# dsforza96/yocto-hair

Measured on AMD Instinct MI355X. Metric: Msamples/sec (whole node), 720x720x1536spp sphere-hairblock; per-pixel L2 vs CPU ref, higher is better.
Workload: dtype f32

## Files before the change

### yocto-hair_amd/csrc/dev_hair.h

```cpp
#ifndef YH_DEV_HAIR_H_
#define YH_DEV_HAIR_H_
#include "dev_math.h"

namespace yhd {

constexpr int p_max = 3;

struct hair_hit {
  float h, gamma_o;
  frame w2b;
};

#ifndef YH_HAIR_FAST
#define YH_HAIR_FAST 1
#endif
#define YH_FAST_DIV YH_HAIR_FAST
#define YH_FAST_EXP 0
#define YH_FAST_LOG YH_HAIR_FAST
#define YH_FAST_TRIG YH_HAIR_FAST
#define YH_FAST_ASIN YH_HAIR_FAST
YH_DEV float h_rcp(float x) { return YH_FAST_DIV ? __builtin_amdgcn_rcpf(x) : 1 / x; }
YH_DEV float h_div(float a, float b) { return YH_FAST_DIV ? a * __builtin_amdgcn_rcpf(b) : a / b; }
YH_DEV float h_div_n(float a, float b) {
  if (!YH_FAST_DIV) return a / b;
// ... 236 lines not shown
  o.pdf0 = ap_pdf[0], o.pdf1 = ap_pdf[1], o.pdf2 = ap_pdf[2], o.pdf3 = ap_pdf[3];
  return o;
}

YH_DEV void hair_eval_pdf_quad(const yhd_material& m, const hair_hit& hh, const hair_out& ho, f3 incoming_,
    f3& f, float& pdf) {
  const int p       = (int)(__lane_id() & 3u);
  f3    incoming    = quad_normalize(transform_vector(hh.w2b, incoming_));
  float sin_theta_o = ho.sin_theta_o, cos_theta_o = ho.cos_theta_o;
  float sin_theta_i = incoming.x;
  float cos_theta_i = exact_safe_sqrt(1 - sqr(sin_theta_i));
  float phi_i       = atan2f(incoming.z, incoming.y);
  float phi         = phi_i - ho.phi_o;
  float sin_theta_op, cos_theta_op;
  tilt(m, p, sin_theta_o, cos_theta_o, sin_theta_op, cos_theta_op);
  if (p < p_max) cos_theta_op = fabs_(cos_theta_op);
  float mpv  = mp(m, p, cos_theta_i, cos_theta_op, sin_theta_i, sin_theta_op);
  float npv  = p < p_max ? np(m, phi, p, hh.gamma_o, ho.gamma_t) : 0.0f;
  const f3    a0 = ho.ap0, a1 = ho.ap1, a2 = ho.ap2, a3 = ho.ap3;
  const float q0 = ho.pdf0, q1 = ho.pdf1, q2 = ho.pdf2, q3 = ho.pdf3;
  const bool  is0 = p == 0, is1 = p == 1, is2 = p == 2;
  f3    apq  = f3{is0 ? a0.x : is1 ? a1.x : is2 ? a2.x : a3.x, is0 ? a0.y : is1 ? a1.y : is2 ? a2.y : a3.y,
      is0 ? a0.z : is1 ? a1.z : is2 ? a2.z : a3.z};
  float appq = is0 ? q0 : is1 ? q1 : is2 ? q2 : q3;
  f3    tf   = p < p_max ? mpv * apq * npv : h_div(mpv * apq, 2 * pif);
  float tp   = p < p_max ? mpv * appq * npv : mpv * appq * (1 / (2 * pif));
  f   = mk3(0.0f);
  pdf = 0.0f;
  f   = f + f3{quad_bcast_f<0>(tf.x), quad_bcast_f<0>(tf.y), quad_bcast_f<0>(tf.z)};
  pdf += quad_bcast_f<0>(tp);
  f   = f + f3{quad_bcast_f<1>(tf.x), quad_bcast_f<1>(tf.y), quad_bcast_f<1>(tf.z)};
  pdf += quad_bcast_f<1>(tp);
  f   = f + f3{quad_bcast_f<2>(tf.x), quad_bcast_f<2>(tf.y), quad_bcast_f<2>(tf.z)};
  pdf += quad_bcast_f<2>(tp);
  f   = f + f3{quad_bcast_f<3>(tf.x), quad_bcast_f<3>(tf.y), quad_bcast_f<3>(tf.z)};
  pdf += quad_bcast_f<3>(tp);
}
YH_DEV void hair_eval_pdf_lane(const yhd_material& m, const hair_hit& hh, const hair_out& ho, f3 incoming_,
    f3& f, float& pdf) {
  f3    incoming    = normalize(transform_vector(hh.w2b, incoming_));
  float sin_theta_o = ho.sin_theta_o, cos_theta_o = ho.cos_theta_o;
  float sin_theta_i = incoming.x;
  float cos_theta_i = exact_safe_sqrt(1 - sqr(sin_theta_i));
  float phi_i       = atan2f(incoming.z, incoming.y);
  float phi         = phi_i - ho.phi_o;
  f   = mk3(0.0f);
  pdf = 0.0f;
  const f3    apv[p_max]  = {ho.ap0, ho.ap1, ho.ap2};
  const float appv[p_max] = {ho.pdf0, ho.pdf1, ho.pdf2};
#pragma unroll
  for (int p = 0; p < p_max; p++) {
    float sin_theta_op, cos_theta_op;
    tilt(m, p, sin_theta_o, cos_theta_o, sin_theta_op, cos_theta_op);
    cos_theta_op = fabs_(cos_theta_op);
    float mpv    = mp(m, p, cos_theta_i, cos_theta_op, sin_theta_i, sin_theta_op);
    float npv    = np(m, phi, p, hh.gamma_o, ho.gamma_t);
    f            = f + mpv * apv[p] * npv;
    pdf += mpv * appv[p] * npv;
  }
  float mpl = mp(m, p_max, cos_theta_i, cos_theta_o, sin_theta_i, sin_theta_o);
  f         = f + h_div(mpl * ho.ap3, 2 * pif);
  pdf += mpl * ho.pdf3 * (1 / (2 * pif));
}
YH_DEV void hair_eval_pdf_quad(const yhd_material& m, const hair_hit& hh, f3 outgoing_, f3 incoming_,
    f3& f, float& pdf) {
  hair_out ho = hair_prepare<true>(m, hh, outgoing_);
  hair_eval_pdf_quad(m, hh, ho, incoming_, f, pdf);
}

YH_DEV uint32_t compact1by1(uint32_t x) {
  x &= 0x55555555;
  x = (x ^ (x >> 1)) & 0x33333333;
  x = (x ^ (x >> 2)) & 0x0f0f0f0f;
  x = (x ^ (x >> 4)) & 0x00ff00ff;
  x = (x ^ (x >> 8)) & 0x0000ffff;
  return x;
}
YH_DEV void demux_float(float f, float& a, float& b) {
  uint64_t v = (uint64_t)(f * 4294967296.0f);
  a          = (float)compact1by1((uint32_t)v) / 65536.0f;
  b          = (float)compact1by1((uint32_t)(v >> 1)) / 65536.0f;
}

YH_DEV f3 hair_sample(const yhd_material& m, const hair_hit& hh, const hair_out& ho, float rnx, float rny) {
  float sin_theta_o = ho.sin_theta_o, cos_theta_o = ho.cos_theta_o, phi_o = ho.phi_o;
  float u00, u01, u10, u11;
  demux_float(rnx, u00, u01);
  demux_float(rny, u10, u11);
  int   p  = 0;
  float u1 = u00 - ho.pdf0, u2 = u1 - ho.pdf1;
  if (!(u00 < ho.pdf0)) p = !(u1 < ho.pdf1) ? (!(u2 < ho.pdf2) ? 3 : 2) : 1;
  float sin_theta_op, cos_theta_op;
  tilt(m, p, sin_theta_o, cos_theta_o, sin_theta_op, cos_theta_op);
  u10 = fmax_(u10, 1e-5f);
  float vp = 0, em2v = 0;
  vp   = p == 0 ? m.v[0] : p == 1 ? m.v[1] : m.v[2];
  em2v = p == 0 ? m.exp_m2_inv_v[0] : p == 1 ? m.exp_m2_inv_v[1] : m.exp_m2_inv_v[2];
  float cos_theta   = 1 + vp * d_log(u10 + (1 - u10) * em2v);
  float sin_theta   = d_safe_sqrt(1 - sqr(cos_theta));
  float cos_phi     = d_cos_turns(u11);
  float sin_theta_i = -cos_theta * sin_theta_op + sin_theta * cos_phi * cos_theta_op;
  float cos_theta_i = d_safe_sqrt(1 - sqr(sin_theta_i));
  float dphi;
  if (p < p_max) {
    float x = -m.s * d_log(d_rcp(u01 * m.tl_norm + m.tl_cdf_a) - 1);
    dphi    = phi_fn(p, hh.gamma_o, ho.gamma_t) + fclamp(x, -pif, pif);
  } else {
    dphi = 2 * pif * u01;
  }
  float phi_i    = phi_o + dphi;
  f3    incoming = f3{sin_theta_i, cos_theta_i * d_cos(phi_i), cos_theta_i * d_sin(phi_i)};
  return d_transform_direction(transpose_rot(hh.w2b), incoming);
}
YH_DEV f3 hair_sample(const yhd_material& m, const hair_hit& hh, f3 outgoing_, float rnx, float rny) {
  hair_out ho = hair_prepare(m, hh, outgoing_);
  return hair_sample(m, hh, ho, rnx, rny);
}

YH_DEV void derive_material(yhd_material& m) {
#pragma unroll
  for (int p = 0; p <= p_max; p++) {
    m.inv_v[p]        = 1 / m.v[p];
    m.log_inv_2v[p]   = logf(1 / (2 * m.v[p]));
    m.exp_m2_inv_v[p] = expf(-2 / m.v[p]);
    m.mp_den[p]       = sinh((double)(1 / m.v[p])) * 2 * m.v[p];
  }
  float cb   = 1 / (1 + expf(-pif / m.s));
  float ca   = 1 / (1 + expf(-(-pif) / m.s));
  m.tl_cdf_a = ca;
  m.tl_norm  = cb - ca;
}

}
#endif
```

### yocto-hair_amd/csrc/dev_path.h

```cpp
#ifndef YH_DEV_PATH_H_
#define YH_DEV_PATH_H_
#include "dev_hair.h"
#include "dev_surface.h"
#include "dev_trace.h"
#if YH_LANE
#include "dev_lane.h"
#endif

namespace yhd {

YH_DEV ray_t sample_camera(const yhd_camera& cam, int i, int j, int w, int h, float pu, float pv,
    float lu, float lv) {
  const unsigned int ql = __lane_id() & 3u;
  float uvq = (ql == 0 ? (float)i + pu : (float)j + pv) / (ql == 0 ? (float)w : (float)h);
  float uvx = quad_bcast_f<0>(uvq), uvy = quad_bcast_f<1>(uvq);
  f3    q  = {cam.film_x * (0.5f - uvx), cam.film_y * (uvy - 0.5f), cam.lens};
  f3    dc = -quad_normalize(q);
  f3    e  = mk3(0.0f);
  if (cam.aperture != 0) {
    float r   = sqrtf(lv);
    float phi = 2 * pif * lu;
    float lx = cosf(phi) * r, ly = sinf(phi) * r;
    e = f3{lx * cam.aperture / 2, ly * cam.aperture / 2, 0};
  }
  f3    p  = quad_div(dc * cam.focus, fabs_(dc.z));
  f3    d  = quad_normalize(p - e);
  frame f  = ldframe(cam.frame);
  return mkray(transform_point(f, e), quad_normalize(transform_vector(f, d)));
}

YH_DEV ray_t sample_camera_lane(const yhd_camera& cam, int i, int j, int w, int h, float pu, float pv, float lu, float lv) {
  float uvx = ((float)i + pu) / (float)w, uvy = ((float)j + pv) / (float)h;
  f3    q   = {cam.film_x * (0.5f - uvx), cam.film_y * (uvy - 0.5f), cam.lens};
  f3    dc  = -normalize(q);
  f3    e   = mk3(0.0f);
  if (cam.aperture != 0) {
    float r   = sqrtf(lv);
    float phi = 2 * pif * lu;
    float lx = cosf(phi) * r, ly = sinf(phi) * r;
    e = f3{lx * cam.aperture / 2, ly * cam.aperture / 2, 0};
  }
  f3    p = (dc * cam.focus) / fabs_(dc.z);
  f3    d = normalize(p - e);
  frame f = ldframe(cam.frame);
  return mkray(transform_point(f, e), normalize(transform_vector(f, d)));
}

YH_DEV f3 transform_normal(const frame& a, f3 b) { return normalize(transform_vector(a, b)); }
YH_DEV f3 quad_transform_normal(const frame& a, f3 b) { return quad_normalize(transform_vector(a, b)); }

YH_DEV f3 eval_position(const yhd_scene& sc, const yhd_object& o, int element, float u, float v) {
  frame    fr = ldframe(o.frame);
  yhd_int4 e  = sc.elems[o.elem_base + element];
  if (o.kind == YH_KIND_TRIANGLES) {
    f3 p0 = xyz(sc.vpos[o.vert_base + e.x]), p1 = xyz(sc.vpos[o.vert_base + e.y]),
       p2 = xyz(sc.vpos[o.vert_base + e.z]);
    return transform_point(fr, p0 * (1 - u - v) + p1 * u + p2 * v);
  } else {
    f3 p0 = xyz(sc.vpos[o.vert_base + e.x]), p1 = xyz(sc.vpos[o.vert_base + e.y]);
    return transform_point(fr, p0 * (1 - u) + p1 * u);
  }
}

struct hit_geom {
  f3 position, normal, element_normal;
};
YH_DEV hit_geom eval_hit(const yhd_scene& sc, const yhd_object& o, int slot, float u, float v) {
  frame    fr = ldframe(o.frame);
  hit_geom g;
  if (o.kind == YH_KIND_TRIANGLES) {
    const yhd_float4* rec = sc.prims + (size_t)o.prim_base + (size_t)slot * 6;
    f3 p0 = xyz(ldg4(rec)), p1 = xyz(ldg4(rec + 1)), p2 = xyz(ldg4(rec + 2));
    g.position       = transform_point(fr, p0 * (1 - u - v) + p1 * u + p2 * v);
    g.element_normal = quad_transform_normal(fr, quad_normalize(cross(p1 - p0, p2 - p0)));
    if (o.has_normals) {
      f3 n0 = xyz(ldg4(rec + 3)), n1 = xyz(ldg4(rec + 4)), n2 = xyz(ldg4(rec + 5));
      g.normal = quad_transform_normal(fr, quad_normalize(n0 * (1 - u - v) + n1 * u + n2 * v));
    } else {
      g.normal = g.element_normal;
    }
  } else {
    const yhd_float4* rec = sc.prims + (size_t)o.prim_base + (size_t)slot * 4;
    f3 p0 = xyz(ldg4(rec)), p1 = xyz(ldg4(rec + 1));
    g.position       = transform_point(fr, p0 * (1 - u) + p1 * u);
    g.element_normal = quad_transform_normal(fr, quad_normalize(p1 - p0));
    if (o.has_normals) {
      f3 n0 = xyz(ldg4(rec + 2)), n1 = xyz(ldg4(rec + 3));
      g.normal = quad_transform_normal(fr, quad_normalize(n0 * (1 - u) + n1 * u));
    } else {
      g.normal = g.element_normal;
    }
  }
  return g;
}

YH_DEV hit_geom eval_hit_fetch_first(const yhd_scene& sc, const yhd_object& o, int slot, float u, float v) {
  const bool        tri = o.kind == YH_KIND_TRIANGLES;
  const yhd_float4* rec = sc.prims + (size_t)o.prim_base + (size_t)slot * (tri ? 6 : 4);
  const v4f r0 = ldg4(rec), r1 = ldg4(rec + 1), r2 = ldg4(rec + 2), r3 = ldg4(rec + 3);
  v4f       r4 = r3, r5 = r3;
  if (tri) r4 = ldg4(rec + 4), r5 = ldg4(rec + 5);
  frame    fr = ldframe(o.frame);
  hit_geom g;
  if (tri) {
    f3 p0 = xyz(r0), p1 = xyz(r1), p2 = xyz(r2);
    g.position       = transform_point(fr, p0 * (1 - u - v) + p1 * u + p2 * v);
    g.element_normal = quad_transform_normal(fr, quad_normalize(cross(p1 - p0, p2 - p0)));
    if (o.has_normals) {
      f3 n0 = xyz(r3), n1 = xyz(r4), n2 = xyz(r5);
      g.normal = quad_transform_normal(fr, quad_normalize(n0 * (1 - u - v) + n1 * u + n2 * v));
    } else {
      g.normal = g.element_normal;
    }
  } else {
    f3 p0 = xyz(r0), p1 = xyz(r1);
    g.position       = transform_point(fr, p0 * (1 - u) + p1 * u);
    g.element_normal = quad_transform_normal(fr, quad_normalize(p1 - p0));
    if (o.has_normals) {
      f3 n0 = xyz(r2), n1 = xyz(r3);
      g.normal = quad_transform_normal(fr, quad_normalize(n0 * (1 - u) + n1 * u));
    } else {
      g.normal = g.element_normal;
    }
  }
  return g;
}

YH_DEV f3 eval_env_texture(const yhd_scene& sc, const yhd_environment& env, float u_, float v_) {
  if (env.tex_w == 0) return mk3(1.0f);
  int   sx = env.tex_w, sy = env.tex_h;
  float s = fmodf(u_, 1.0f) * sx;
  if (s < 0) s += sx;
  float t = fmodf(v_, 1.0f) * sy;
  if (t < 0) t += sy;
  int   i = iclamp((int)s, 0, sx - 1), j = iclamp((int)t, 0, sy - 1);
  int   ii = (i + 1) % sx, jj = (j + 1) % sy;
  float u = s - i, v = t - j;
  const yhd_float4* tx = sc.env_texels + env.texel_base;
  f3 a = xyz(tx[(size_t)j * sx + i]), b = xyz(tx[(size_t)jj * sx + i]);
  f3 c = xyz(tx[(size_t)j * sx + ii]), d = xyz(tx[(size_t)jj * sx + ii]);
  return a * (1 - u) * (1 - v) + b * (1 - u) * v + c * u * (1 - v) + d * u * v;
}
template <bool COUNT, bool CENV = false>
YH_DEV f3 eval_environment(const trace_ctx& tc, f3 dir, const const_env_t* ce = nullptr) {
  const yhd_scene& sc = *tc.sc;
  f3 emission = mk3(0.0f);
  if constexpr (CENV) {
    if (COUNT)
      for (int k = 0; k < sc.num_environments; k++) count_quad<COUNT>(tc.stats->envl);
    return ld3(ce->env_sum);
  }
  for (int k = 0; k < sc.num_environments; k++) {
    const yhd_environment& env = sc.environments[k];
    if (COUNT) count_quad<COUNT>(tc.stats->envl);
    if (env.tex_w == 0) {
      emission = emission + ld3(env.emission) * mk3(1.0f);
      continue;
    }
    f3    wl = transform_direction(ldframe(env.inv_frame), dir);
    float tx = atan2f(wl.z, wl.x) / (2 * pif);
    float ty = acosf(fclamp(wl.y, -1.0f, 1.0f)) / pif;
    if (tx < 0) tx += 1;
    emission = emission + ld3(env.emission) * eval_env_texture(sc, env, tx, ty);
  }
  return emission;
}

YH_DEV void const_environments(const yhd_scene& sc, const_env_t& ce) {
  f3 emission = mk3(0.0f);
  for (int k = 0; k < sc.num_environments; k++) emission = emission + ld3(sc.environments[k].emission) * mk3(1.0f);
  float pdf = 0.0f;
  for (int k = 0; k < sc.num_lights; k++) pdf += 1 / (4 * pif);
  pdf *= (float)1 / (float)sc.num_lights;
  auto uniform = [](float v) { return __int_as_float(__builtin_amdgcn_readfirstlane(__float_as_int(v))); };
  ce.env_sum[0] = uniform(emission.x), ce.env_sum[1] = uniform(emission.y), ce.env_sum[2] = uniform(emission.z);
  ce.lights_pdf = uniform(pdf);
}

template <typename P>
YH_DEV int cdf_upper_bound(P cdf, int lo, int len, float r) {
  while (len > 0) {
    int half = len >> 1;
    if (!(r < cdf[lo + half])) {
      lo += half + 1;
      len -= half + 1;
    } else {
      len = half;
    }
  }
  return lo;
}
template <typename P>
YH_DEV int sample_discrete_cdf(P cdf, int n, float r) {
  float back = cdf[n - 1];
  r          = fclamp(r * back, 0.0f, back - 0.00001f);
  return iclamp(cdf_upper_bound(cdf, 0, n, r), 0, n - 1);
}
YH_DEV int sample_discrete_cdf_indexed(const float* cdf, int n, const YH_LDS float* tab, int K, int S, float r) {
  float back = tab[K - 1];
  r          = fclamp(r * back, 0.0f, back - 0.00001f);
  int k      = cdf_upper_bound(tab, 0, K, r);
  if (k >= K) return n - 1;
  int lo = k * S;
  return iclamp(cdf_upper_bound(cdf, lo, min(S, n - lo), r), 0, n - 1);
}

YH_DEV void object_frames(const trace_ctx& tc, int object, frame& fr, frame& inv) {
  if (tc.lds_scene) {
    const YH_LDS v4f* ob = tc.lds_scene + YH_OBJECT_F4 * object;
    v4f a = ob[0], b = ob[1], c = ob[2], d = ob[3], e = ob[4], g = ob[5];
    fr.x = {a.x, a.y, a.z}, fr.y = {a.w, b.x, b.y}, fr.z = {b.z, b.w, c.x}, fr.o = {c.y, c.z, c.w};
    inv.x = {d.x, d.y, d.z}, inv.y = {d.w, e.x, e.y}, inv.z = {e.z, e.w, g.x}, inv.o = {g.y, g.z, g.w};
  } else {
    const yhd_object& o = tc.sc->objects[object];
    fr = ldframe(o.frame), inv = ldframe(o.inv_frame);
  }
}
YH_DEV bool small_light_hit(const YH_LDS v4f* L, const frame& inv, f3 ro, f3 rd, int& slot, float& uu, float& vv) {
  f3  lo = transform_point(inv, ro), ld = transform_vector(inv, rd);
  f3  ldinv = quad_rcp(ld);
  v4f b0 = L[0], b1 = L[1];
  if (!intersect_bbox(lo, ldinv, ray_eps, flt_max, xyz(b0), xyz(b1))) return false;
  const int num  = __float_as_int(b0.w);
  float     tmax = flt_max;
  bool      hit  = false;
  for (int i = 0; i < num; i++) {
    float u = 0, v = 0, d = 0;
    if (intersect_triangle(lo, ld, ray_eps, tmax, xyz(L[2 + 3 * i]), xyz(L[3 + 3 * i]), xyz(L[4 + 3 * i]), u, v, d)) hit = true, slot = i, uu = u, vv = v, tmax = d;
  }
  return hit;
}

template <bool COUNT, bool BIG_LIGHTS, bool CENV = false>
YH_DEV f3 sample_lights(const trace_ctx& tc, f3 position, float rl, float rel, float ruvx,
    float ruvy) {
  const yhd_scene& sc = *tc.sc;
  if constexpr (CENV) {
    float z   = 2 * ruvy - 1;
    float r   = sqrtf(fclamp(1 - z * z, 0.0f, 1.0f));
    float phi = 2 * pif * ruvx;
    return f3{r * cosf(phi), r * sinf(phi), z};
  }
  int n        = sc.num_lights;
  int light_id = iclamp((int)(rl * n), 0, n - 1);
  const yhd_light& light = sc.lights[light_id];
  if (light.object >= 0 && (!BIG_LIGHTS || (light.small_base >= 0 && tc.lds_lights))) {
    const YH_LDS v4f* L = tc.lds_lights + light.small_base;
    int   element = sample_discrete_cdf((const YH_LDS float*)(L + 14), light.cdf_count, rel);
    int   rec     = 0;
    for (int i = 1; i < __float_as_int(L[0].w); i++)
      if (__float_as_int(L[2 + 3 * i].w) == element) rec = i;
    float su = sqrtf(ruvx);
    float u = 1 - su, v = ruvy * su;
    frame fr, inv;
    object_frames(tc, light.object, fr, inv);
    f3 p0 = xyz(L[2 + 3 * rec]), p1 = xyz(L[3 + 3 * rec]), p2 = xyz(L[4 + 3 * rec]);
    f3 lposition = transform_point(fr, p0 * (1 - u - v) + p1 * u + p2 * v);
    return normalize(lposition - position);
  } else if (BIG_LIGHTS && light.object >= 0) {
    int   element = sample_discrete_cdf(sc.light_cdf + light.cdf_base, light.cdf_count, rel);
    float su      = sqrtf(ruvx);
    float u = 1 - su, v = ruvy * su;
    f3 lposition = eval_position(sc, sc.objects[light.object], element, u, v);
    return normalize(lposition - position);
  } else if (light.environment >= 0) {
    const yhd_environment& env = sc.environments[light.environment];
    if (env.tex_w) {
      if (COUNT) count_quad<COUNT>(tc.stats->envs);
      int   idx = (tc.lds_envtab && light_id == sc.env_tab_light)
                      ? sample_discrete_cdf_indexed(sc.light_cdf + light.cdf_base, light.cdf_count, tc.lds_envtab, sc.env_tab_k, sc.env_tab_stride, rel)
                      : sample_discrete_cdf(sc.light_cdf + light.cdf_base, light.cdf_count, rel);
      float ux  = (idx % env.tex_w + 0.5f) / env.tex_w;
      float uy  = (idx / env.tex_w + 0.5f) / env.tex_h;
      return transform_direction(ldframe(env.frame),
          f3{cosf(ux * 2 * pif) * sinf(uy * pif), cosf(uy * pif), sinf(ux * 2 * pif) * sinf(uy * pif)});
    } else {
      float z   = 2 * ruvy - 1;
      float r   = sqrtf(fclamp(1 - z * z, 0.0f, 1.0f));
      float phi = 2 * pif * ruvx;
      return f3{r * cosf(phi), r * sinf(phi), z};
    }
  }
  return mk3(0.0f);
}

template <bool COUNT, int STRIDE, bool BIG_LIGHTS, bool CENV = false>
YH_DEV float sample_lights_pdf(const trace_ctx& tc, f3 position, f3 direction, const const_env_t* ce = nullptr) {
  const yhd_scene& sc = *tc.sc;
  float pdf = 0.0f;
  if constexpr (CENV) return ce->lights_pdf;
  for (int k = 0; k < sc.num_lights; k++) {
    const yhd_light& light = sc.lights[k];
    if (light.object >= 0 && (!BIG_LIGHTS || (light.small_base >= 0 && tc.lds_lights))) {
      const YH_LDS v4f* L = tc.lds_lights + light.small_base;
      frame fr, inv;
      object_frames(tc, light.object, fr, inv);
      const float area = L[1].w;
      float lpdf = 0.0f;
      f3    next_position = position;
      for (int bounce = 0; bounce < 100; bounce++) {
        int   slot = 0;
        float uu = 0, vv = 0;
        if (!small_light_hit(L, inv, next_position, direction, slot, uu, vv)) break;
        f3 p0 = xyz(L[2 + 3 * slot]), p1 = xyz(L[3 + 3 * slot]), p2 = xyz(L[4 + 3 * slot]);
        f3 lposition = transform_point(fr, p0 * (1 - uu - vv) + p1 * uu + p2 * vv);
        f3 lnormal   = quad_transform_normal(fr, quad_normalize(cross(p1 - p0, p2 - p0)));
        f3 dp        = lposition - position;
        lpdf += dot(dp, dp) / (fabs_(dot(lnormal, direction)) * area);
        next_position = lposition + direction * 1e-3f;
      }
      pdf += lpdf;
    } else if (BIG_LIGHTS && light.object >= 0) {
      const yhd_object& o = sc.objects[light.object];
      float lpdf = 0.0f;
      f3    next_position = position;
      for (int bounce = 0; bounce < 100; bounce++) {
        hit_t isec;
#if YH_LANE
        isec = lane_trace(tc, *tc.ls, next_position, direction, light.object);
#else
        isec = trace_ray<COUNT, STRIDE>(tc, mkray(next_position, direction), light.object);
#endif
        if (isec.object < 0) break;
        hit_geom lg        = eval_hit(sc, o, isec.slot, isec.u, isec.v);
        f3       lposition = lg.position;
        f3       lnormal   = lg.element_normal;
        float area      = sc.light_cdf[light.cdf_base + light.cdf_count - 1];
        f3    dp        = lposition - position;
        lpdf += dot(dp, dp) / (fabs_(dot(lnormal, direction)) * area);
        next_position = lposition + direction * 1e-3f;
      }
      pdf += lpdf;
    } else if (light.environment >= 0) {
      const yhd_environment& env = sc.environments[light.environment];
      if (env.tex_w) {
        f3    wl = transform_direction(ldframe(env.inv_frame), direction);
        float tx = atan2f(wl.z, wl.x) / (2 * pif);
        float ty = acosf(fclamp(wl.y, -1.0f, 1.0f)) / pif;
        if (tx < 0) tx += 1;
        int   i   = iclamp((int)(tx * env.tex_w), 0, env.tex_w - 1);
        int   j   = iclamp((int)(ty * env.tex_h), 0, env.tex_h - 1);
        int   idx = j * env.tex_w + i;
        const float* cdf = sc.light_cdf + light.cdf_base;
        float prob = (idx == 0 ? cdf[0] : cdf[idx] - cdf[idx - 1]) / cdf[light.cdf_count - 1];
        float angle = (2 * pif / env.tex_w) * (pif / env.tex_h) * sinf(pif * (j + 0.5f) / env.tex_h);
        pdf += prob / angle;
      } else {
        pdf += 1 / (4 * pif);
      }
    }
  }
  pdf *= (float)1 / (float)sc.num_lights;
  return pdf;
}

#if YH_LANE
struct lane_lights_pdf_result {
  float pdf;
  int   base;
// ... 137 lines not shown
        f3 c = {fclamp(base.x, 0.0001f, 1.0f), fclamp(base.y, 0.0001f, 1.0f), fclamp(base.z, 0.0001f, 1.0f)};
        ps.medium.density = -f3{logf(c.x), logf(c.y), logf(c.z)} / mat.trdepth;
      }
    } else {
      ps.medium.density = ld3(mat.vol_density);
    }
    ps.medium.scatter    = ld3(mat.vol_scatter) * eval_texture(sc, mat.scattering_tex, false, tu, tv);
    ps.medium.anisotropy = mat.vol_anisotropy;
#if YH_LANE
    ps.medium_mem[0] = yhd_float4{ps.medium.density.x, ps.medium.density.y, ps.medium.density.z, ps.medium.anisotropy};
    ps.medium_mem[1] = yhd_float4{ps.medium.scatter.x, ps.medium.scatter.y, ps.medium.scatter.z, 0.0f};
#endif
  }
  ps.in_medium = !ps.in_medium;
}

template <bool COUNT, int STRIDE, bool GENERAL, bool TRIM = false, bool CENV = false>
YH_DEV bool path_step(const trace_ctx& tc, path_t& ps, const hit_t& isec, rng_t& rng, int bounces, const const_env_t* ce = nullptr) {
  static_assert(!TRIM || (!GENERAL && !YH_LANE), "the trimmed shading pass exists for the plain quad kernels");
  static_assert(!CENV || TRIM, "the constant-environment form exists for the trimmed kernels");
  const yhd_scene& sc = *tc.sc;
  unsigned long long k0 = 0, k1 = 0, k2 = 0, k3 = 0;
  if (COUNT) k0 = clock64();
#if YH_LANE
  if (isec.object < 0) return false;
#else
  if (isec.object < 0) {
    YH_REGION_MARK("miss");
    unsigned long long km = 0;
    if (COUNT) km = clock64();
    ps.radiance = ps.radiance + ps.weight * eval_environment<COUNT, CENV>(tc, ps.ray.d, ce);
    if (COUNT) tc.stats->c_rest += clock64() - k0;
    count_region<COUNT>(tc.stats, YH_REGION_MISS, km);
    return false;
  }
#endif
  unsigned long long kr = 0;
  if (COUNT) kr = clock64();
  YH_REGION_MARK("fetch");
  f3 outgoing = -ps.ray.d;
  if (GENERAL && ps.in_medium) {
#if YH_LANE
    {
      const yhd_float4 m0 = ps.medium_mem[0], m1 = ps.medium_mem[1];
      ps.medium.density = f3{m0.x, m0.y, m0.z}, ps.medium.anisotropy = m0.w, ps.medium.scatter = f3{m1.x, m1.y, m1.z};
    }
#endif
    float rd = rand1f(rng), rl = rand1f(rng);
    float dist = sample_transmittance(ps.medium.density, isec.distance, rl, rd);
    ps.weight  = ps.weight * (eval_transmittance(ps.medium.density, dist) /
                                sample_transmittance_pdf(ps.medium.density, dist, isec.distance));
    if (dist < isec.distance) {
      f3 position = ps.ray.o + ps.ray.d * dist;
      ps.hit      = true;
      f3 incoming;
      if (rand1f(rng) < 0.5f) {
        float rnx = rand1f(rng), rny = rand1f(rng);
        float rnl = rand1f(rng);
        (void)rnl;
        incoming = sample_scattering(ps.medium, outgoing, rnx, rny);
      } else {
        float ruvx = rand1f(rng), ruvy = rand1f(rng);
        float rel = rand1f(rng);
        float rl2 = rand1f(rng);
        incoming  = sample_lights<COUNT, GENERAL>(tc, position, rl2, rel, ruvx, ruvy);
      }
      f3    f         = eval_scattering(ps.medium, outgoing, incoming);
      float pdf       = sample_scattering_pdf(ps.medium, outgoing, incoming);
#if YH_LANE
      float light_pdf = lane_lights_pdf<GENERAL>(tc, position, incoming);
#else
      float light_pdf = sample_lights_pdf<COUNT, STRIDE, GENERAL>(tc, position, incoming);
#endif
      ps.weight = ps.weight * (f / (0.5f * pdf + 0.5f * light_pdf));
      ps.ray    = mkray(position, incoming);
      if (COUNT) tc.stats->c_rest += clock64() - k0;
      return path_continue(ps, rng, bounces);
    }
  }
  constexpr bool from_lds = (!GENERAL && (YH_LANE || STRIDE != 64)) || TRIM;
  const yhd_object&   o   = !from_lds ? sc.objects[isec.object] : *(const yhd_object*)(const YH_LDS yhd_object*)(tc.lds_scene + YH_OBJECT_F4 * isec.object);
  const yhd_material& mat = !from_lds ? sc.materials[o.material] : *(const yhd_material*)(const YH_LDS yhd_material*)(tc.lds_mats + YH_MATERIAL_F4 * o.material);
  hit_geom hg;
  if constexpr (TRIM) hg = eval_hit_fetch_first(sc, o, isec.slot, isec.u, isec.v);
  else hg = eval_hit(sc, o, isec.slot, isec.u, isec.v);
  f3 position = hg.position;
  f3 nrm      = hg.normal;
  hit_maps hm;
  if constexpr (GENERAL) hm = eval_hit_maps(sc, o, isec, !mat.plain, nrm);
  f3 normal;
  bool is_hair = o.kind == YH_KIND_LINES;
  if (is_hair) {
    normal = quad_orthonormalize(outgoing, nrm);
  } else {
    normal = (!mat.thin || dot(nrm, outgoing) >= 0) ? nrm : -nrm;
  }
  if (COUNT) count_quad<COUNT>(is_hair ? tc.stats->hair : tc.stats->surf);
  const bool     general = GENERAL && !mat.plain;
  surface_brdf_t sb;
  float          tu = isec.u, tv = isec.v, etex_x = 1.0f;
  f3             ctex = mk3(1.0f), etex = mk3(1.0f);
  if (general) {
    if constexpr (GENERAL) tu = hm.tu, tv = hm.tv;
    if (mat.color_tex >= 0 || mat.emission_tex >= 0 || mat.scattering_tex >= 0) {
      if constexpr (GENERAL) {
        if (!hm.have_tc) eval_texcoord(sc, o, isec, tu, tv);
      }
      ctex = eval_texture(sc, mat.color_tex, false, tu, tv);
      if (mat.emission_tex >= 0) {
        etex   = eval_texture(sc, mat.emission_tex, false, tu, tv);
        etex_x = eval_texture(sc, mat.emission_tex, true, tu, tv).x;
      }
    }
    if constexpr (GENERAL) sb = surface_brdf(mat, normal, outgoing, ctex, etex_x, hm.f);
    else sb = surface_brdf(mat, normal, outgoing, ctex, etex_x);
    if (sb.opacity < 1 && rand1f(rng) >= sb.opacity) {
      ps.ray = mkray(position + ps.ray.d * 1e-2f, ps.ray.d);
      if (COUNT) tc.stats->c_rest += clock64() - k0;
      return true;
    }
  }
  ps.hit      = true;
  ps.radiance = ps.radiance + ps.weight * (ld3(mat.emission) * etex);
  if (general && is_delta(sb)) {
    f3    incoming = surface_sample_delta(sb, normal, outgoing, rand1f(rng));
    f3    brdfcos;
    float pdf;
    surface_eval_pdf_delta(sb, normal, outgoing, incoming, brdfcos, pdf);
    ps.weight = ps.weight * (brdfcos / pdf);
    medium_crossing(sc, ps, mat, normal, outgoing, incoming, ctex, etex_x, tu, tv);
    ps.ray    = mkray(position, incoming);
    if (COUNT) tc.stats->c_rest += clock64() - k0;
    return path_continue(ps, rng, bounces);
  }
  count_region<COUNT>(tc.stats, YH_REGION_FETCH, kr);
  YH_REGION_MARK("hair");
  hair_hit hh;
  hair_out ho;
  if (is_hair) {
    hh = hair_setup<!YH_LANE>(isec.v, normal, nrm);
    ho = hair_prepare<!YH_LANE>(mat, hh, outgoing);
  }
  count_region<COUNT>(tc.stats, YH_REGION_HAIR, kr, is_hair);
  YH_REGION_MARK("sample");

  if (COUNT) k1 = clock64(), tc.stats->c_geom += k1 - k0;
  f3 incoming;
  if (rand1f(rng) < 0.5f) {
    float rnx = rand1f(rng), rny = rand1f(rng);
    float rnl = rand1f(rng);
    if (is_hair) {
      incoming = hair_sample(mat, hh, ho, rnx, rny);
    } else if (general) {
      incoming = surface_sample(sb, normal, outgoing, rnl, rnx, rny);
    } else {
      incoming = mk3(0.0f);
      if (mat.diffuse_pdf != 0 && rnl < 0.0f + mat.diffuse_pdf) {
        if (!(dot(normal, outgoing) <= 0)) incoming = TRIM ? sample_hemisphere_cos_quad(normal, rnx, rny) : sample_hemisphere_cos(normal, rnx, rny);
      }
    }
  } else {
    float ruvx = rand1f(rng), ruvy = rand1f(rng);
    float rel = rand1f(rng);
    float rl  = rand1f(rng);
    incoming  = sample_lights<COUNT, GENERAL, CENV>(tc, position, rl, rel, ruvx, ruvy);
  }
  if (COUNT) k2 = clock64(), tc.stats->c_sample += k2 - k1;
  count_region<COUNT>(tc.stats, YH_REGION_SAMPLE, kr);
  YH_REGION_MARK("eval");
  f3    brdfcos;
  float brdf_pdf;
  if (is_hair) {
#if YH_LANE
    hair_eval_pdf_lane(mat, hh, ho, incoming, brdfcos, brdf_pdf);
#else
    hair_eval_pdf_quad(mat, hh, ho, incoming, brdfcos, brdf_pdf);
#endif
  } else if (general) {
    surface_eval_pdf(sb, normal, outgoing, incoming, brdfcos, brdf_pdf);
  } else {
    brdfcos  = mk3(0.0f);
    brdf_pdf = 0.0f;
    f3 diffuse = ld3(mat.color);
    bool below = dot(normal, incoming) <= 0 || dot(normal, outgoing) <= 0;
    if (!is_zero(diffuse)) {
      f3 lobe = below ? mk3(0.0f) : mk3(1.0f) / pif * dot(normal, incoming);
      brdfcos = brdfcos + diffuse * lobe;
    }
    if (mat.diffuse_pdf != 0) {
      float lobe = 0.0f;
      if (!below) {
        float cosw = dot(normal, incoming);
        lobe       = (cosw <= 0) ? 0 : cosw / pif;
      }
      brdf_pdf += mat.diffuse_pdf * lobe;
    }
  }
  if (COUNT) k3 = clock64(), tc.stats->c_eval += k3 - k2;
  count_region<COUNT>(tc.stats, YH_REGION_EVAL, kr);
  YH_REGION_MARK("lights_pdf");
#if YH_LANE
  float light_pdf = lane_lights_pdf<GENERAL>(tc, position, incoming);
#else
  float light_pdf = sample_lights_pdf<COUNT, STRIDE, GENERAL, CENV>(tc, position, incoming, ce);
#endif
  count_region<COUNT>(tc.stats, YH_REGION_LIGHTS_PDF, kr);
  YH_REGION_MARK("weight");
  if constexpr (TRIM) ps.weight = ps.weight * quad_div(brdfcos, 0.5f * brdf_pdf + 0.5f * light_pdf);
  else ps.weight = ps.weight * (brdfcos / (0.5f * brdf_pdf + 0.5f * light_pdf));
  if (general) medium_crossing(sc, ps, mat, normal, outgoing, incoming, ctex, etex_x, tu, tv);
  ps.ray    = mkray(position, incoming);
  if (COUNT) tc.stats->c_rest += clock64() - k3;
  const bool goes_on = path_continue(ps, rng, bounces);
  count_region<COUNT>(tc.stats, YH_REGION_WEIGHT, kr);
  return goes_on;
}

template <bool COUNT, int STRIDE, int SHADER>
YH_DEV bool shade_step(const trace_ctx& tc, path_t& ps, const hit_t& isec, rng_t& rng, int bounces) {
  const yhd_scene& sc = *tc.sc;
  if (isec.object < 0) {
    f3 env = eval_environment<COUNT>(tc, ps.ray.d);
    if (SHADER == YH_SHADER_NORMAL) ps.radiance = env, ps.hit = true;
    else ps.radiance = ps.radiance + ps.weight * env;
    return false;
  }
  f3 outgoing = -ps.ray.d;
  const yhd_object&   o   = sc.objects[isec.object];
  const yhd_material& mat = sc.materials[o.material];
  hit_geom hg = eval_hit(sc, o, isec.slot, isec.u, isec.v);
  f3   position = hg.position, nrm = hg.normal;
  const hit_maps hm = eval_hit_maps(sc, o, isec, true, nrm);
  bool is_hair  = o.kind == YH_KIND_LINES;
  f3   normal   = is_hair ? quad_orthonormalize(outgoing, nrm) : ((!mat.thin || dot(nrm, outgoing) >= 0) ? nrm : -nrm);
  if (SHADER == YH_SHADER_NORMAL) {
    ps.radiance = normal * 0.5f + mk3(0.5f), ps.hit = true;
    return false;
  }
  if (COUNT) count_quad<COUNT>(is_hair ? tc.stats->hair : tc.stats->surf);
  float tu = hm.tu, tv = hm.tv, etex_x = 1.0f;
  f3    ctex = mk3(1.0f), etex = mk3(1.0f);
// ... 74 lines not shown
```

### yocto-hair_amd/csrc/dev_surface.h

```cpp
#ifndef YH_DEV_SURFACE_H_
#define YH_DEV_SURFACE_H_
#include "dev_hair.h"
#include "dev_math.h"

namespace yhd {

YH_DEV f3 reflect(f3 w, f3 n) { return -w + 2 * dot(n, w) * n; }
YH_DEV f3 refract(f3 w, f3 n, float inv_eta) {
  float cosine = dot(n, w);
  float k      = 1 + inv_eta * inv_eta * (cosine * cosine - 1);
  if (k < 0) return mk3(0.0f);
  return -w * inv_eta + (inv_eta * cosine - sqrtf(k)) * n;
}

YH_DEV float fresnel_dielectric(float eta, f3 normal, f3 outgoing) {
  return fresnel_dielectric_cos(eta, dot(normal, outgoing));
}
YH_DEV float conductor_channel(float eta, float etak, float cosw, float cos2, float sin2) {
  float eta2 = eta * eta, etak2 = etak * etak;
  float t0       = eta2 - etak2 - sin2;
  float a2plusb2 = sqrtf(t0 * t0 + 4 * eta2 * etak2);
  float t1       = a2plusb2 + cos2;
  float a        = sqrtf((a2plusb2 + t0) / 2);
  float t2       = 2 * a * cosw;
  float rs       = (t1 - t2) / (t1 + t2);
  float t3       = cos2 * a2plusb2 + sin2 * sin2;
  float t4       = t2 * sin2;
  float rp       = rs * (t3 - t4) / (t3 + t4);
  return (rp + rs) / 2;
}
YH_DEV f3 fresnel_conductor(f3 eta, f3 etak, f3 normal, f3 outgoing) {
  float cosw = dot(normal, outgoing);
  if (cosw <= 0) return mk3(0.0f);
  cosw       = fclamp(cosw, -1.0f, 1.0f);
  float cos2 = cosw * cosw;
  float sin2 = fclamp(1 - cos2, 0.0f, 1.0f);
  return {conductor_channel(eta.x, etak.x, cosw, cos2, sin2), conductor_channel(eta.y, etak.y, cosw, cos2, sin2),
      conductor_channel(eta.z, etak.z, cosw, cos2, sin2)};
}

YH_DEV float microfacet_distribution(float roughness, f3 normal, f3 halfway) {
  float cosine = dot(normal, halfway);
  if (cosine <= 0) return 0;
  float roughness2 = roughness * roughness;
  float cosine2    = cosine * cosine;
  return roughness2 / (pif * (cosine2 * roughness2 + 1 - cosine2) * (cosine2 * roughness2 + 1 - cosine2));
}
YH_DEV float microfacet_shadowing1(float roughness, f3 normal, f3 halfway, f3 direction) {
  float cosine  = dot(normal, direction);
  float cosineh = dot(halfway, direction);
  if (cosine * cosineh <= 0) return 0;
  float roughness2 = roughness * roughness;
  float cosine2    = cosine * cosine;
  return 2 * fabs_(cosine) / (fabs_(cosine) + sqrtf(cosine2 - roughness2 * cosine2 + roughness2));
}
YH_DEV float microfacet_shadowing(float roughness, f3 normal, f3 halfway, f3 outgoing, f3 incoming) {
  return microfacet_shadowing1(roughness, normal, halfway, outgoing) *
         microfacet_shadowing1(roughness, normal, halfway, incoming);
}
YH_DEV f3 from_local_z(f3 normal, f3 local) {
  f3    zz   = normalize(normal);
  float sign = copysignf(1.0f, zz.z);
  float a    = -1.0f / (sign + zz.z);
  float b    = zz.x * zz.y * a;
  f3    x    = {1.0f + sign * zz.x * zz.x * a, sign * b, -sign * zz.x};
  f3    y    = {b, sign + zz.y * zz.y * a, -zz.y};
  return normalize(x * local.x + y * local.y + zz * local.z);
}
YH_DEV f3 sample_microfacet(float roughness, f3 normal, float rx, float ry) {
  float phi   = 2 * pif * rx;
  float theta = atanf(roughness * sqrtf(ry / (1 - ry)));
  float st = sinf(theta), ct = cosf(theta);
  return from_local_z(normal, f3{cosf(phi) * st, sinf(phi) * st, ct});
}
YH_DEV float sample_microfacet_pdf(float roughness, f3 normal, f3 halfway) {
  float cosine = dot(normal, halfway);
  if (cosine < 0) return 0;
  return microfacet_distribution(roughness, normal, halfway) * cosine;
}
YH_DEV f3 sample_hemisphere_cos(f3 normal, float rx, float ry) {
  float z   = sqrtf(ry);
  float r   = sqrtf(1 - z * z);
  float phi = 2 * pif * rx;
  return from_local_z(normal, f3{r * cosf(phi), r * sinf(phi), z});
}
YH_DEV f3 sample_hemisphere_cos_quad(f3 normal, float rx, float ry) {
  float z   = sqrtf(ry);
  float r   = sqrtf(1 - z * z);
  float phi = 2 * pif * rx;
  f3    local = f3{r * cosf(phi), r * sinf(phi), z};
  f3    zz   = quad_normalize(normal);
  float sign = copysignf(1.0f, zz.z);
  float a    = -1.0f / (sign + zz.z);
  float b    = zz.x * zz.y * a;
  f3    x    = {1.0f + sign * zz.x * zz.x * a, sign * b, -sign * zz.x};
  f3    y    = {b, sign + zz.y * zz.y * a, -zz.y};
  return quad_normalize(x * local.x + y * local.y + zz * local.z);
}
YH_DEV bool both_above(f3 normal, f3 outgoing, f3 incoming) {
  return !(dot(normal, incoming) <= 0 || dot(normal, outgoing) <= 0);
}

YH_DEV f3 eval_diffuse_reflection(f3 normal, f3 outgoing, f3 incoming) {
  if (!both_above(normal, outgoing, incoming)) return mk3(0.0f);
  return mk3(1.0f) / pif * dot(normal, incoming);
}
YH_DEV float sample_diffuse_reflection_pdf(f3 normal, f3 outgoing, f3 incoming) {
  if (!both_above(normal, outgoing, incoming)) return 0;
  float cosw = dot(normal, incoming);
  return (cosw <= 0) ? 0 : cosw / pif;
}
YH_DEV f3 sample_diffuse_reflection(f3 normal, f3 outgoing, float rx, float ry) {
  if (dot(normal, outgoing) <= 0) return mk3(0.0f);
  return sample_hemisphere_cos(normal, rx, ry);
}
YH_DEV f3 microfacet_reflection_with(f3 F, float roughness, f3 normal, f3 halfway, f3 outgoing, f3 incoming) {
  float D = microfacet_distribution(roughness, normal, halfway);
  float G = microfacet_shadowing(roughness, normal, halfway, outgoing, incoming);
  return F * D * G / (4 * dot(normal, outgoing) * dot(normal, incoming)) * dot(normal, incoming);
}
YH_DEV f3 eval_microfacet_reflection(float ior, float roughness, f3 normal, f3 outgoing, f3 incoming) {
  if (!both_above(normal, outgoing, incoming)) return mk3(0.0f);
  f3    halfway = normalize(incoming + outgoing);
  float f       = fresnel_dielectric(ior, halfway, incoming);
  return microfacet_reflection_with(mk3(1.0f) * f, roughness, normal, halfway, outgoing, incoming);
}
YH_DEV f3 eval_microfacet_reflection(f3 eta, f3 etak, float roughness, f3 normal, f3 outgoing, f3 incoming) {
  if (!both_above(normal, outgoing, incoming)) return mk3(0.0f);
  f3 halfway = normalize(incoming + outgoing);
  return microfacet_reflection_with(fresnel_conductor(eta, etak, halfway, incoming), roughness, normal, halfway,
      outgoing, incoming);
}
YH_DEV float sample_microfacet_reflection_pdf(float roughness, f3 normal, f3 outgoing, f3 incoming) {
  if (!both_above(normal, outgoing, incoming)) return 0;
  f3 halfway = normalize(outgoing + incoming);
  return sample_microfacet_pdf(roughness, normal, halfway) / (4 * fabs_(dot(outgoing, halfway)));
}
YH_DEV f3 sample_microfacet_reflection(float roughness, f3 normal, f3 outgoing, float rx, float ry) {
  if (dot(normal, outgoing) <= 0) return mk3(0.0f);
  return reflect(outgoing, sample_microfacet(roughness, normal, rx, ry));
}
YH_DEV f3 eval_microfacet_transmission(float roughness, f3 normal, f3 outgoing, f3 incoming) {
  if (dot(normal, incoming) >= 0 || dot(normal, outgoing) <= 0) return mk3(0.0f);
  f3    reflected = reflect(-incoming, normal);
  f3    halfway   = normalize(reflected + outgoing);
  float D         = microfacet_distribution(roughness, normal, halfway);
  float G         = microfacet_shadowing(roughness, normal, halfway, outgoing, reflected);
  return mk3(1.0f) * D * G / (4 * dot(normal, outgoing) * dot(normal, reflected)) * (dot(normal, reflected));
}
YH_DEV float sample_microfacet_transmission_pdf(float roughness, f3 normal, f3 outgoing, f3 incoming) {
  if (dot(normal, incoming) >= 0 || dot(normal, outgoing) <= 0) return 0;
  f3    reflected = reflect(-incoming, normal);
  f3    halfway   = normalize(reflected + outgoing);
  float d         = sample_microfacet_pdf(roughness, normal, halfway);
  return d / (4 * fabs_(dot(outgoing, halfway)));
}
YH_DEV f3 sample_microfacet_transmission(float roughness, f3 normal, f3 outgoing, float rx, float ry) {
  if (dot(normal, outgoing) <= 0) return mk3(0.0f);
  f3 reflected = reflect(outgoing, sample_microfacet(roughness, normal, rx, ry));
  return -reflect(reflected, normal);
}
struct refraction_side {
  bool  entering;
  f3    up_normal;
  float rel_ior;
};
YH_DEV refraction_side refraction_setup(float ior, f3 normal, f3 outgoing) {
  refraction_side s;
  s.entering  = dot(normal, outgoing) >= 0;
  s.up_normal = s.entering ? normal : -normal;
  s.rel_ior   = s.entering ? ior : (1 / ior);
  return s;
}
YH_DEV f3 eval_microfacet_refraction(float ior, float roughness, f3 normal, f3 outgoing, f3 incoming) {
  refraction_side s = refraction_setup(ior, normal, outgoing);
  if (dot(normal, incoming) * dot(normal, outgoing) >= 0) {
    f3    halfway = normalize(incoming + outgoing);
    float F       = fresnel_dielectric(s.rel_ior, halfway, outgoing);
    float D       = microfacet_distribution(roughness, s.up_normal, halfway);
    float G       = microfacet_shadowing(roughness, s.up_normal, halfway, outgoing, incoming);
// ... 296 lines not shown
```

Baseline: 2729.

## Overlap hit-record loads with RNG draws and share one sincos tail across samplers

Splits hit-geometry evaluation into an issue step and a use step. In the TRIM path, the random numbers are drawn between the two steps, fenced by sched_barrier, so global load latency is hidden behind RNG arithmetic. The hair, hemisphere and sphere-light samplers now return angles only, and a single merged cos/sin tail builds the direction, so divergent branches no longer each carry their own trig. The RNG draws are reordered: the branch choice, then three uniforms up front, then the light uniform, which changes the random stream relative to before. The scheduling fences and empty asm constraints may also raise register pressure.

```diff
diff --git a/yocto-hair_amd/csrc/dev_hair.h b/yocto-hair_amd/csrc/dev_hair.h
--- a/yocto-hair_amd/csrc/dev_hair.h
+++ b/yocto-hair_amd/csrc/dev_hair.h
@@ -342,7 +342,8 @@
   b          = (float)compact1by1((uint32_t)(v >> 1)) / 65536.0f;
 }
 
-YH_DEV f3 hair_sample(const yhd_material& m, const hair_hit& hh, const hair_out& ho, float rnx, float rny) {
+YH_DEV void hair_sample_angle(const yhd_material& m, const hair_hit& hh, const hair_out& ho, float rnx, float rny, float& phi_i,
+    float& cos_theta_i, float& sin_theta_i) {
   float sin_theta_o = ho.sin_theta_o, cos_theta_o = ho.cos_theta_o, phi_o = ho.phi_o;
   float u00, u01, u10, u11;
   demux_float(rnx, u00, u01);
@@ -359,8 +360,8 @@
   float cos_theta   = 1 + vp * d_log(u10 + (1 - u10) * em2v);
   float sin_theta   = d_safe_sqrt(1 - sqr(cos_theta));
   float cos_phi     = d_cos_turns(u11);
-  float sin_theta_i = -cos_theta * sin_theta_op + sin_theta * cos_phi * cos_theta_op;
-  float cos_theta_i = d_safe_sqrt(1 - sqr(sin_theta_i));
+  sin_theta_i       = -cos_theta * sin_theta_op + sin_theta * cos_phi * cos_theta_op;
+  cos_theta_i       = d_safe_sqrt(1 - sqr(sin_theta_i));
   float dphi;
   if (p < p_max) {
     float x = -m.s * d_log(d_rcp(u01 * m.tl_norm + m.tl_cdf_a) - 1);
@@ -368,9 +369,15 @@
   } else {
     dphi = 2 * pif * u01;
   }
-  float phi_i    = phi_o + dphi;
-  f3    incoming = f3{sin_theta_i, cos_theta_i * d_cos(phi_i), cos_theta_i * d_sin(phi_i)};
-  return d_transform_direction(transpose_rot(hh.w2b), incoming);
+  phi_i = phi_o + dphi;
+}
+YH_DEV f3 hair_sample_finish(const hair_hit& hh, float sin_theta_i, float y, float z) {
+  return d_transform_direction(transpose_rot(hh.w2b), f3{sin_theta_i, y, z});
+}
+YH_DEV f3 hair_sample(const yhd_material& m, const hair_hit& hh, const hair_out& ho, float rnx, float rny) {
+  float phi_i, cos_theta_i, sin_theta_i;
+  hair_sample_angle(m, hh, ho, rnx, rny, phi_i, cos_theta_i, sin_theta_i);
+  return hair_sample_finish(hh, sin_theta_i, cos_theta_i * d_cos(phi_i), cos_theta_i * d_sin(phi_i));
 }
 YH_DEV f3 hair_sample(const yhd_material& m, const hair_hit& hh, f3 outgoing_, float rnx, float rny) {
   hair_out ho = hair_prepare(m, hh, outgoing_);
diff --git a/yocto-hair_amd/csrc/dev_path.h b/yocto-hair_amd/csrc/dev_path.h
--- a/yocto-hair_amd/csrc/dev_path.h
+++ b/yocto-hair_amd/csrc/dev_path.h
@@ -94,36 +94,50 @@
   return g;
 }
 
-YH_DEV hit_geom eval_hit_fetch_first(const yhd_scene& sc, const yhd_object& o, int slot, float u, float v) {
+struct hit_rows {
+  v4f   r0, r1, r2, r3, r4, r5;
+  frame fr;
+};
+YH_DEV hit_rows hit_rows_issue(const yhd_scene& sc, const yhd_object& o, int slot) {
   const bool        tri = o.kind == YH_KIND_TRIANGLES;
   const yhd_float4* rec = sc.prims + (size_t)o.prim_base + (size_t)slot * (tri ? 6 : 4);
-  const v4f r0 = ldg4(rec), r1 = ldg4(rec + 1), r2 = ldg4(rec + 2), r3 = ldg4(rec + 3);
-  v4f       r4 = r3, r5 = r3;
-  if (tri) r4 = ldg4(rec + 4), r5 = ldg4(rec + 5);
-  frame    fr = ldframe(o.frame);
+  hit_rows h;
+  h.r0 = ldg4(rec), h.r1 = ldg4(rec + 1), h.r2 = ldg4(rec + 2), h.r3 = ldg4(rec + 3);
+  h.r4 = h.r5 = v4f{0, 0, 0, 0};
+  if (tri) h.r4 = ldg4(rec + 4), h.r5 = ldg4(rec + 5);
+  h.fr = ldframe(o.frame);
+  return h;
+}
+YH_DEV hit_geom hit_rows_use(const yhd_object& o, const hit_rows& h, float u, float v) {
+  const bool   tri = o.kind == YH_KIND_TRIANGLES;
+  const frame& fr  = h.fr;
+  asm volatile("" ::"v"(h.r0.w), "v"(h.r1.w), "v"(h.r2.w), "v"(h.r3.w), "v"(h.r4.w), "v"(h.r5.w));
   hit_geom g;
   if (tri) {
-    f3 p0 = xyz(r0), p1 = xyz(r1), p2 = xyz(r2);
+    f3 p0 = xyz(h.r0), p1 = xyz(h.r1), p2 = xyz(h.r2);
     g.position       = transform_point(fr, p0 * (1 - u - v) + p1 * u + p2 * v);
     g.element_normal = quad_transform_normal(fr, quad_normalize(cross(p1 - p0, p2 - p0)));
     if (o.has_normals) {
-      f3 n0 = xyz(r3), n1 = xyz(r4), n2 = xyz(r5);
+      f3 n0 = xyz(h.r3), n1 = xyz(h.r4), n2 = xyz(h.r5);
       g.normal = quad_transform_normal(fr, quad_normalize(n0 * (1 - u - v) + n1 * u + n2 * v));
     } else {
       g.normal = g.element_normal;
     }
   } else {
-    f3 p0 = xyz(r0), p1 = xyz(r1);
+    f3 p0 = xyz(h.r0), p1 = xyz(h.r1);
     g.position       = transform_point(fr, p0 * (1 - u) + p1 * u);
     g.element_normal = quad_transform_normal(fr, quad_normalize(p1 - p0));
     if (o.has_normals) {
-      f3 n0 = xyz(r2), n1 = xyz(r3);
+      f3 n0 = xyz(h.r2), n1 = xyz(h.r3);
       g.normal = quad_transform_normal(fr, quad_normalize(n0 * (1 - u) + n1 * u));
     } else {
       g.normal = g.element_normal;
     }
   }
   return g;
+}
+YH_DEV hit_geom eval_hit_fetch_first(const yhd_scene& sc, const yhd_object& o, int slot, float u, float v) {
+  return hit_rows_use(o, hit_rows_issue(sc, o, slot), u, v);
 }
 
 YH_DEV f3 eval_env_texture(const yhd_scene& sc, const yhd_environment& env, float u_, float v_) {
@@ -231,11 +245,27 @@
   return hit;
 }
 
-template <bool COUNT, bool BIG_LIGHTS, bool CENV = false>
+struct angle_tail {
+  int   kind;
+  float phi, radius, third;
+};
+enum { YH_TAIL_NONE = 0, YH_TAIL_SPHERE, YH_TAIL_HEMISPHERE, YH_TAIL_HAIR };
+YH_DEV void sample_sphere_angle(float ruvx, float ruvy, angle_tail& t) {
+  float z  = 2 * ruvy - 1;
+  t.radius = sqrtf(fclamp(1 - z * z, 0.0f, 1.0f));
+  t.phi    = 2 * pif * ruvx;
+  t.third  = z;
+  t.kind   = YH_TAIL_SPHERE;
+}
+template <bool COUNT, bool BIG_LIGHTS, bool CENV = false, bool SPLIT = false>
 YH_DEV f3 sample_lights(const trace_ctx& tc, f3 position, float rl, float rel, float ruvx,
-    float ruvy) {
+    float ruvy, angle_tail* tail = nullptr) {
   const yhd_scene& sc = *tc.sc;
   if constexpr (CENV) {
+    if constexpr (SPLIT) {
+      sample_sphere_angle(ruvx, ruvy, *tail);
+      return mk3(0.0f);
+    }
     float z   = 2 * ruvy - 1;
     float r   = sqrtf(fclamp(1 - z * z, 0.0f, 1.0f));
     float phi = 2 * pif * ruvx;
@@ -275,6 +305,10 @@
       return transform_direction(ldframe(env.frame),
           f3{cosf(ux * 2 * pif) * sinf(uy * pif), cosf(uy * pif), sinf(ux * 2 * pif) * sinf(uy * pif)});
     } else {
+      if constexpr (SPLIT) {
+        sample_sphere_angle(ruvx, ruvy, *tail);
+        return mk3(0.0f);
+      }
       float z   = 2 * ruvy - 1;
       float r   = sqrtf(fclamp(1 - z * z, 0.0f, 1.0f));
       float phi = 2 * pif * ruvx;
@@ -578,8 +612,19 @@
   const yhd_object&   o   = !from_lds ? sc.objects[isec.object] : *(const yhd_object*)(const YH_LDS yhd_object*)(tc.lds_scene + YH_OBJECT_F4 * isec.object);
   const yhd_material& mat = !from_lds ? sc.materials[o.material] : *(const yhd_material*)(const YH_LDS yhd_material*)(tc.lds_mats + YH_MATERIAL_F4 * o.material);
   hit_geom hg;
-  if constexpr (TRIM) hg = eval_hit_fetch_first(sc, o, isec.slot, isec.u, isec.v);
-  else hg = eval_hit(sc, o, isec.slot, isec.u, isec.v);
+  float    rbranch = 0, rs0 = 0, rs1 = 0, rs2 = 0;
+  if constexpr (TRIM) {
+    const hit_rows rows = hit_rows_issue(sc, o, isec.slot);
+    __builtin_amdgcn_sched_barrier(0);
+    rbranch = rand1f(rng);
+    rs0 = rand1f(rng), rs1 = rand1f(rng);
+    rs2 = rand1f(rng);
+    asm volatile("" : "+v"(rbranch), "+v"(rs0), "+v"(rs1), "+v"(rs2), "+v"(rng.state));
+    __builtin_amdgcn_sched_barrier(0);
+    hg = hit_rows_use(o, rows, isec.u, isec.v);
+  } else {
+    hg = eval_hit(sc, o, isec.slot, isec.u, isec.v);
+  }
   f3 position = hg.position;
   f3 nrm      = hg.normal;
   hit_maps hm;
@@ -642,7 +687,31 @@
 
   if (COUNT) k1 = clock64(), tc.stats->c_geom += k1 - k0;
   f3 incoming;
-  if (rand1f(rng) < 0.5f) {
+  if constexpr (TRIM) {
+    angle_tail at;
+    at.kind = YH_TAIL_NONE, at.phi = 0, at.radius = 0, at.third = 0;
+    incoming = mk3(0.0f);
+    if (rbranch < 0.5f) {
+      if (is_hair) {
+        hair_sample_angle(mat, hh, ho, rs0, rs1, at.phi, at.radius, at.third);
+        at.kind = YH_TAIL_HAIR;
+      } else if (mat.diffuse_pdf != 0 && rs2 < 0.0f + mat.diffuse_pdf) {
+        if (!(dot(normal, outgoing) <= 0)) {
+          sample_hemisphere_cos_angle(rs0, rs1, at.phi, at.radius, at.third);
+          at.kind = YH_TAIL_HEMISPHERE;
+        }
+      }
+    } else {
+      float rl = rand1f(rng);
+      incoming = sample_lights<COUNT, GENERAL, CENV, true>(tc, position, rl, rs2, rs0, rs1, &at);
+    }
+    if (at.kind != YH_TAIL_NONE) {
+      const float y = at.radius * cosf(at.phi), z = at.radius * sinf(at.phi);
+      if (at.kind == YH_TAIL_HAIR) incoming = hair_sample_finish(hh, at.third, y, z);
+      else if (at.kind == YH_TAIL_HEMISPHERE) incoming = from_local_z_quad(normal, f3{y, z, at.third});
+      else incoming = f3{y, z, at.third};
+    }
+  } else if (rand1f(rng) < 0.5f) {
     float rnx = rand1f(rng), rny = rand1f(rng);
     float rnl = rand1f(rng);
     if (is_hair) {
@@ -652,7 +721,7 @@
     } else {
       incoming = mk3(0.0f);
       if (mat.diffuse_pdf != 0 && rnl < 0.0f + mat.diffuse_pdf) {
-        if (!(dot(normal, outgoing) <= 0)) incoming = TRIM ? sample_hemisphere_cos_quad(normal, rnx, rny) : sample_hemisphere_cos(normal, rnx, rny);
+        if (!(dot(normal, outgoing) <= 0)) incoming = sample_hemisphere_cos(normal, rnx, rny);
       }
     }
   } else {
diff --git a/yocto-hair_amd/csrc/dev_surface.h b/yocto-hair_amd/csrc/dev_surface.h
--- a/yocto-hair_amd/csrc/dev_surface.h
+++ b/yocto-hair_amd/csrc/dev_surface.h
@@ -84,11 +84,12 @@
   float phi = 2 * pif * rx;
   return from_local_z(normal, f3{r * cosf(phi), r * sinf(phi), z});
 }
-YH_DEV f3 sample_hemisphere_cos_quad(f3 normal, float rx, float ry) {
-  float z   = sqrtf(ry);
-  float r   = sqrtf(1 - z * z);
-  float phi = 2 * pif * rx;
-  f3    local = f3{r * cosf(phi), r * sinf(phi), z};
+YH_DEV void sample_hemisphere_cos_angle(float rx, float ry, float& phi, float& r, float& z) {
+  z   = sqrtf(ry);
+  r   = sqrtf(1 - z * z);
+  phi = 2 * pif * rx;
+}
+YH_DEV f3 from_local_z_quad(f3 normal, f3 local) {
   f3    zz   = quad_normalize(normal);
   float sign = copysignf(1.0f, zz.z);
   float a    = -1.0f / (sign + zz.z);
@@ -96,6 +97,11 @@
   f3    x    = {1.0f + sign * zz.x * zz.x * a, sign * b, -sign * zz.x};
   f3    y    = {b, sign + zz.y * zz.y * a, -zz.y};
   return quad_normalize(x * local.x + y * local.y + zz * local.z);
+}
+YH_DEV f3 sample_hemisphere_cos_quad(f3 normal, float rx, float ry) {
+  float phi, r, z;
+  sample_hemisphere_cos_angle(rx, ry, phi, r, z);
+  return from_local_z_quad(normal, f3{r * cosf(phi), r * sinf(phi), z});
 }
 YH_DEV bool both_above(f3 normal, f3 outgoing, f3 incoming) {
   return !(dot(normal, incoming) <= 0 || dot(normal, outgoing) <= 0);
```

Result: no change. 2756 (median of 4 runs) (+1.0%).
